# shicaiwei123/ICCV2025-GDL

Measured on AMD Instinct MI355X. Metric: audio-visual samples/sec, CREMA-D DGL train step (whole job), higher is better.
Workload: dtype bf16; 1 GPU; CREMA-D DGL (main_dgl.py, ConcatFusion_DGL) ResNet18 a+v, spec 1x257x188 + frames 3x3x224x224, alpha=4, SGD lr 2e-3 mom .9 wd 1e-4, clip 40; per_gpu_batch=64, global_batch=64, parallelism=dp1, buckets=none

## Files before the change

iccv2025-gdl_amd/csrc/api.cpp:

```cpp
#include "ops.h"

using namespace gdl;

#ifdef GDL_TIMING
namespace gdl { extern unsigned long long* g_timing_buf; }
#endif
extern "C" {
GDL_API int gdl_debug_timing_buffer(void* buf) {
#ifdef GDL_TIMING
    gdl::g_timing_buf = (unsigned long long*)buf;
    return GDL_OK;
#else
    (void)buf;
    return GDL_ERR_ARG;
#endif
}


const char* gdl_last_error(void) { return last_error(); }
int gdl_version(void) { return 100; }

int gdl_device_info(int* cu_count, char* name, int name_len) {
    int dev = 0;
    hipError_t e = hipGetDevice(&dev);
// ... 14 lines not shown
    return conv_tiles_m(dtype, N, H, W, C, K, R, S, stride, pad);
}

size_t gdl_conv_table_bytes(int mode, int N, int H, int W, int R, int S, int stride, int pad) {
    return gather_table_bytes(mode, N, H, W, R, S, stride, pad);
}
int gdl_conv_build_table(int mode, int dtype, int N, int H, int W, int C, int K, int R, int S, int stride, int pad,
                         void* table, void* stream) {
    GDL_REQUIRE(dt_ok(dtype) && table && (mode == GATHER_FWD || mode == GATHER_DGRAD), "conv_build_table: bad arguments");
    return build_gather_table(mode, dtype, N, H, W, C, K, R, S, stride, pad, (GatherEntry*)table, (hipStream_t)stream);
}
int gdl_conv_fwd(int dtype, const void* x, const void* w_krsc, void* y, float* bn_partial, const void* table, int N, int H,
                 int W, int C, int K, int R, int S, int stride, int pad, void* stream) {
    GDL_REQUIRE(x && w_krsc && y, "conv_fwd: null pointer");
    return conv_fwd(dtype, x, w_krsc, y, bn_partial, table, N, H, W, C, K, R, S, stride, pad, (hipStream_t)stream);
}
int gdl_bn_act_bits(int dtype, const void* y, const float* scale, const float* shift, const void* res, const float* res_scale,
                    const float* res_shift, void* out, uint8_t* relu_bits, size_t M, int C, void* stream) {
    GDL_REQUIRE(dt_ok(dtype) && y && scale && shift && out && relu_bits, "bn_act_bits: bad arguments");
    return bn_act(dtype, y, scale, shift, res, res_scale, res_shift, 1, out, M, C, (hipStream_t)stream, relu_bits);
}
int gdl_conv_dgrad_relu(int dtype, const void* dy, const void* w_crsk, void* dx, const void* addend, const uint8_t* relu_bits,
                        const void* table, int N, int H, int W, int C, int K, int R, int S, int stride, int pad, void* stream) {
    GDL_REQUIRE(dy && w_crsk && dx && relu_bits, "conv_dgrad_relu: null pointer");
    return conv_dgrad(dtype, dy, w_crsk, dx, addend, table, N, H, W, C, K, R, S, stride, pad, (hipStream_t)stream, relu_bits);
}
int gdl_conv_fwd_bias(int dtype, const void* x, const void* w_krsc, void* y, const float* bias, const void* addend, void* gelu_out,
                      const void* table, int N, int H, int W, int C, int K, int R, int S, int stride, int pad, void* stream) {
    GDL_REQUIRE(x && w_krsc && y, "conv_fwd_bias: null pointer");
    return conv_fwd_bias(dtype, x, w_krsc, y, bias, addend, gelu_out, table, N, H, W, C, K, R, S, stride, pad, (hipStream_t)stream);
// ... 628 lines not shown
```

iccv2025-gdl_amd/csrc/conv_igemm.hip:

```cpp
#include <stdlib.h>

#include <type_traits>

#include "bnacc.h"
#include "common.h"
#include "gather.h"
#include "ops.h"
#include "prof.h"

#include <hip/hip_ext.h>

namespace gdl {

struct ConvArgs {
    const void* in;
    const void* wt;
    void* out;
    const void* addend;
    const float* bias;
    void* gelu_out;
    const void* gelu_u;
    const uint8_t* relu_bits;
    float* stats;
    BnAcc sacc;
// ... 1048 lines not shown
        d[0] = acc_wait;
        d[1] = acc_issue;
        d[2] = acc_rd;
        d[3] = acc_m0;
        d[4] = acc_m1;
        d[5] = (unsigned long long)kpt * a.ntaps;
    }
#endif
}

#include "conv_pslab.h"

constexpr int C64_BM = 128;
constexpr int C64_GRID = 512;
constexpr int C64_F32_TILE = 35 * 1024;
template <int MODE, bool BW = false, bool ADD = false>
__global__ __launch_bounds__(256, 2) void conv3x3_c64_kernel(ConvArgs a) {
    static_assert(!BW || MODE == MODE_DGRAD, "BW: data gradient only");
    static_assert(!ADD || MODE == MODE_DGRAD, "ADD: data gradient only");
    constexpr bool STATS = MODE == MODE_FWD;
    extern __shared__ __attribute__((aligned(16))) unsigned char smem[];
    constexpr int BM = C64_BM, PITCH = 64 * 2 + 16;
    const int tid = threadIdx.x, lane = tid & 63, wave = __builtin_amdgcn_readfirstlane(tid >> 6);
    const int wm = wave & 1, wn = wave >> 1;
    const int frow = lane & 15, fg = lane >> 4;
    GDL_STAMP(0);
    const int xcd = blockIdx.x & 7, bj = blockIdx.x >> 3, bpx = gridDim.x >> 3;
    const int mt_per_xcd = (a.mtiles + 7) >> 3;
    const int t_end = min(a.mtiles, (xcd + 1) * mt_per_xcd);
    int tile = xcd * mt_per_xcd + bj;
    const int nins = (a.slab_rows + 7) >> 3;
    const int slab_bytes = BW ? max(nins * 1024, C64_F32_TILE) : nins * 1024;
    const unsigned smem_base = lds_addr(smem);
    const int nbuf = a.single_slab ? 1 : 2;
    const unsigned zrow = smem_base + nbuf * slab_bytes;
    const __amdgpu_buffer_rsrc_t rin = __builtin_amdgcn_make_buffer_rsrc((void*)a.in, 0, a.in_bytes, 0x00020000);

    typedef unsigned u32x4_t __attribute__((ext_vector_type(4)));
    u32x4_t wreg[9][2][2];
    {
        const __amdgpu_buffer_rsrc_t rwt = __builtin_amdgcn_make_buffer_rsrc((void*)a.wt, 0, a.wt_bytes, 0x00020000);
        for (int p = wave; p < 72; p += 4) {
            const int row = p * 8 + (lane >> 3);
            dma16(rwt, smem + p * 1024, row * 128 + (((lane & 7) ^ swz128(row)) << 4));
        }
        asm volatile("s_waitcnt vmcnt(0)" ::: "memory");
        __builtin_amdgcn_s_barrier();
        asm volatile("" ::: "memory");
#pragma unroll
        for (int tap = 0; tap < 9; ++tap)
#pragma unroll
            for (int h = 0; h < 2; ++h)
#pragma unroll
                for (int n = 0; n < 2; ++n) {
                    const int row = (wn * 32 + n * 16 + frow) * 9 + tap;
                    const unsigned ad = smem_base + row * 128 + (((h * 4 + fg) ^ swz128(row)) << 4);
                    asm volatile("ds_read_b128 %0, %1" : "=v"(wreg[tap][h][n]) : "v"(ad));
                }
        asm volatile("s_waitcnt lgkmcnt(0)" ::: "memory");
        __builtin_amdgcn_s_barrier();
        asm volatile("" ::: "memory");
    }
    if constexpr (BW) {
        if (tid < 128) ((float*)(smem + nbuf * slab_bytes + 1024))[tid] = tid < 64 ? a.bw_mean[tid] : a.bw_rstd[tid - 64];
        ((float*)(smem + nbuf * slab_bytes + 1536))[tid] = 0.f;
        ((float*)(smem + nbuf * slab_bytes + 1536))[tid + 256] = 0.f;
    }
    if (wave == 0) dma16(rin, smem + nbuf * slab_bytes, (int)0x80000000);
    auto load_slab = [&](int sbuf, int m0) {
        unsigned char* dst = smem + sbuf * slab_bytes;
        int ln = lane;
        asm volatile("" : "+v"(ln));
        for (int jj = wave; jj < nins; jj += 4) {
            const int sr = jj * 8 + (ln >> 3);
            const int pix = m0 - (a.W + 1) + sr;
            const bool ok = sr < a.slab_rows && (unsigned)pix < (unsigned)a.in_pixels;
            const int v = ok ? pix * 128 + (((ln & 7) ^ swz128(sr)) << 4) : (int)0x80000000;
            dma16(rin, dst + jj * 1024, v);
        }
    };
    auto load_masks = [&](int m0, unsigned (&fm)[4]) {
#pragma unroll
        for (int m = 0; m < 4; ++m) {
            const int mm = m0 + wm * 64 + m * 16 + frow;
            fm[m] = mm < a.M ? a.table[mm].mask : 0u;
        }
    };
    const int prow0 = wm * 64 + frow + (a.W + 1);
    unsigned zb[4];
#pragma unroll
    for (int m = 0; m < 4; ++m) zb[m] = zrow - 2048u * m;
    const int ec = tid & 7, er0 = tid >> 3;
    float tsum[8], tsq[8];
#pragma unroll
    for (int e = 0; e < 8; ++e) tsum[e] = tsq[e] = 0.f;
    bf16* __restrict__ gout = (bf16*)a.out;
    const bf16* __restrict__ gadd = ADD ? (const bf16*)a.addend : nullptr;
    const uint8_t* __restrict__ rbits = MODE == MODE_DGRAD ? a.relu_bits : nullptr;

    unsigned fmask[4] = {0u, 0u, 0u, 0u};
// ... 21 lines not shown
    GDL_STAMP(1);
#else
#define C64_SEG(i)
#endif
    for (int it = 0; tile < t_end; ++it, tile += bpx) {
#ifdef GDL_TIMING
        tq_a = __builtin_amdgcn_s_memtime();
        ++tq_n;
#endif
        const int m0 = tile * BM;
        const bool more = tile + bpx < t_end;
        const int sb = nbuf == 2 ? (it & 1) : 0;
        if (more && nbuf == 2) {
            load_slab(sb ^ 1, (tile + bpx) * BM);
        }
        C64_SEG(0)
        const unsigned slab = smem_base + sb * slab_bytes;
        f32x4_t acc[2][4];
#pragma unroll
        for (int n = 0; n < 2; ++n)
#pragma unroll
            for (int m = 0; m < 4; ++m) acc[n][m] = f32x4_t{0.f, 0.f, 0.f, 0.f};
        constexpr int NPX = STATS ? 1 : 2;
        uint4 px[NPX][4];
        unsigned pb[4];
        auto tap_addr = [&](int tap) __attribute__((always_inline)) {
            const int sr0 = prow0 + a.pshift[tap];
            const unsigned ad0 = slab + sr0 * 128 + ((fg ^ swz128(sr0)) << 4);
#pragma unroll
            for (int m = 0; m < 4; ++m) pb[m] = ((fmask[m] >> tap) & 1u) ? ad0 : zb[m];
// ... 261 lines not shown
                red[(wave * 64 + lane * 8 + e) * 2 + 1] = ssq[e];
            }
        }
        __syncthreads();
        if (tid < 128) {
            const int c = tid >> 1, w = tid & 1;
            const float s2 = ((red[(0 * 64 + c) * 2 + w] + red[(1 * 64 + c) * 2 + w]) + red[(2 * 64 + c) * 2 + w]) +
                             red[(3 * 64 + c) * 2 + w];
            if (a.sacc.acc)
                bn_acc_add(a.sacc, c, w, s2);
            else
                st_agent(sdst + ((size_t)blockIdx.x * 64 + c) * 2 + w, s2);
        }
    }
    GDL_STAMP(3);
}

static size_t slab_lds_bytes(int BM, int BN, int W, int IC, int dtype, bool single = false) {
    const int bke = dtype == GDL_BF16 ? 64 : 32, esz = dtype == GDL_BF16 ? 2 : 4;
    const int rows = BM + 2 * W + 2;
    const size_t slab = (size_t)((rows + 7) / 8) * 1024;
    const size_t main = 2 * (size_t)BN * 128 + ((IC / bke > 1 && !single) ? 2 : 1) * slab + ((rows & 7) ? 0 : 1024);
    const size_t epi = (size_t)BM * (BN * esz + 16) + 8 * (size_t)BN * 2 * 4;
    return main > epi ? main : epi;
}

struct TileCfg {
    int bm, bn;
};

// ... 21 lines not shown
    int split;
    int rows;
};
struct ConvOpts {
    const void* addend = nullptr;
    float* stats = nullptr;
    const uint8_t* relu_bits = nullptr;
    const void* dy_ds = nullptr;
    const void* w_ds = nullptr;
    const float* bias = nullptr;
    void* gelu_out = nullptr;
    const void* gelu_u = nullptr;
    const BwdStats* bw = nullptr;
    const BnAcc* sacc = nullptr;
    const SplitWs* split = nullptr;
};

static size_t c64_lds_bytes(int W, bool single = false) {
    const size_t b = (single ? 1 : 2) * (size_t)((C64_BM + 2 * W + 2 + 7) / 8) * 1024 + 1024 + 512 + 2048;
    return b > (size_t)72 * 1024 ? b : (size_t)72 * 1024;
}
static constexpr long slab_big_min() { return 128; }
static constexpr long slab_bn128_min() { return 384; }
constexpr int SPLITK_BLOCKS = 200;
static_assert(SPLITK_BLOCKS <= PS_GRID, "split-K blocks");
static int pslab_mode() {
    static int v = -1;
    if (v < 0) {
        const char* e = tune_env("GDL_PSLAB");
        v = e ? atoi(e) : 2;
// ... 164 lines not shown
        if (need > lds) lds = need;
        GDL_REQUIRE(lds <= (size_t)80 * 1024, "conv: LDS of the 64-channel data gradient with BatchNorm sums");
    }
    auto kfn = conv3x3_c64_kernel<MODE, BW, ADD>;
    static DevOnce attr_set;
    if (!attr_set) {
        hipError_t e = hipFuncSetAttribute((const void*)kfn, hipFuncAttributeMaxDynamicSharedMemorySize, 80 * 1024);
        if (e != hipSuccess) return check_hip(e, "hipFuncSetAttribute(conv3x3_c64)");
        attr_set = true;
    }
    static char pname[64] = "";
    if (!pname[0]) snprintf(pname, sizeof(pname), BW ? "gdl::conv3x3_c64_kernel<%d, true>" : "gdl::conv3x3_c64_kernel<%d>", MODE);
    ProfScope prof(pname, PROF_MFMA, st, a.flops, true, a.hbm_bytes);
    hipExtLaunchKernelGGL(kfn, dim3(C64_GRID), dim3(256), lds, st, prof.e0(), prof.e1(), 0, a);
    GDL_CHECK_LAUNCH("conv3x3_c64_kernel");
    return GDL_OK;
}

template <typename T, int MODE>
static int launch_mode(ConvArgs& a, const ConvPlan& pl, hipStream_t st) {
    constexpr bool BF = std::is_same<T, bf16>::value;
    switch (pl.kind) {
        case ConvKind::C64:
            if constexpr (BF) return launch_c64<MODE>(a, pl.lds, st);
            break;
        case ConvKind::PSLAB:
            if constexpr (BF) {
                if (pl.nslab == 1) return pl.bm == 192 ? launch_pslab<3, MODE, false>(a, pl, st) : launch_pslab<2, MODE, false>(a, pl, st);
                return pl.bm == 192 ? launch_pslab<3, MODE, true>(a, pl, st) : launch_pslab<2, MODE, true>(a, pl, st);
            }
// ... 210 lines not shown
    } else {
        a.IC = K;
        a.OC = C;
        a.in_bytes = (unsigned)((size_t)N * P * Q * K * esz);
    }
    a.wt_bytes = (unsigned)((size_t)K * C * R * S * esz);
    GDL_REQUIRE(a.IC % bke == 0, "conv: gather channels %d not a multiple of %d", a.IC, bke);
    GDL_REQUIRE(a.OC % 64 == 0, "conv: output channels %d not a multiple of 64", a.OC);
    GDL_REQUIRE(a.M < (1 << 24), "conv: M = %d exceeds 2^24", a.M);
    if (a.plain && !o.stats && !sacc && !o.relu_bits && !bw && !o.gelu_u && !o.dy_ds &&
        linear_stream_ok(dtype, a.M, a.IC, a.OC, o.addend != nullptr))
        return linear_stream_fwd(in, wt, out, o.addend, o.bias, o.gelu_out, a.M, a.IC, a.OC, st);
    ConvPlan pl;
    rc = plan_conv(pl, mode, dtype, N, H, W, C, K, R, S, stride, pad, o);
    if (rc) return rc;
    a.flops = 2.0 * (double)N * P * Q * K * C * R * S;
    {
        const double esz = dtype == GDL_BF16 ? 2.0 : 4.0;
        a.hbm_bytes = esz * ((double)N * H * W * C + (double)N * P * Q * K + (double)K * C * R * S);
    }
    if (o.dy_ds) {
        GDL_REQUIRE(mode == GATHER_DGRAD && stride == 2 && R == 3 && S == 3 && pad == 1 && o.w_ds && pl.kind == ConvKind::FLAT,
                    "conv: the folded downsample branch needs the 3x3 stride-2 pad-1 data gradient");
        a.in2 = o.dy_ds;
        a.wt2 = o.w_ds;
        a.in2_bytes = a.in_bytes;
        a.wt2_bytes = (unsigned)((size_t)K * C * esz);
        a.flops += 2.0 * (double)N * P * Q * K * C;
    }
    if (mode == GATHER_DGRAD && stride == 2) {
// ... 29 lines not shown
        f.bw_y = a.bw_y, f.bw_mean = a.bw_mean, f.bw_rstd = a.bw_rstd, f.bw_partial = a.bw_partial;
        f.bw_y2 = a.bw_y2, f.bw_mean2 = a.bw_mean2, f.bw_rstd2 = a.bw_rstd2, f.bw_partial2 = a.bw_partial2;
        ProfScope prof("gdl::splitk_finish_kernel", PROF_HBM, st, (double)a.M * a.OC * (4.0 * ks + 2.0 * (1 + (a.addend ? 1 : 0) + (a.bw_y ? 1 : 0) + (a.bw_y2 ? 1 : 0))));
        hipLaunchKernelGGL(splitk_finish_kernel<bf16>, dim3(mt, a.OC / 64), dim3(256), 0, st, f);
        GDL_CHECK_LAUNCH("splitk_finish_kernel");
        if (pl.rows > mt) {
            const size_t off = (size_t)mt * a.OC * 2, n = (size_t)(pl.rows - mt) * a.OC * 2 * sizeof(float);
            for (float* p : {a.stats, a.bw_partial, a.bw_y2 ? a.bw_partial2 : (float*)nullptr})
                if (p) {
                    hipError_t e = hipMemsetAsync(p + off, 0, n, st);
                    if (e != hipSuccess) return check_hip(e, "hipMemsetAsync(split-K partial rows)");
                }
        }
        return GDL_OK;
    }
    if (dtype == GDL_BF16)
        return mode == GATHER_FWD ? launch_mode<bf16, MODE_FWD>(a, pl, st) : launch_mode<bf16, MODE_DGRAD>(a, pl, st);
    return mode == GATHER_FWD ? launch_mode<float, MODE_FWD>(a, pl, st) : launch_mode<float, MODE_DGRAD>(a, pl, st);
}

int conv_fwd(int dtype, const void* x, const void* w, void* y, float* bn_partial, const void* table, int N, int H, int W,
             int C, int K, int R, int S, int stride, int pad, hipStream_t st, const BnAcc* sacc, const SplitWs* split) {
    ConvOpts o;
    o.stats = bn_partial, o.sacc = sacc, o.split = split;
    return run_conv(GATHER_FWD, dtype, x, w, y, table, N, H, W, C, K, R, S, stride, pad, st, o);
}

int stem_taps(int dtype);
int stem_ic(int dtype);
static bool stem_rows(int dtype, int W) {
    static int v = -1;
    if (v < 0) {
        const char* e = tune_env("GDL_STEM_ROWS_FWD");
        v = e ? atoi(e) : 1;
    }
    return v != 0 && dtype == GDL_BF16 && (W - 1) / 2 + 1 >= 64;
}
static bool stem_pers() {
    static int v = -1;
    if (v < 0) {
// ... 124 lines not shown
```

iccv2025-gdl_amd/csrc/encoder.cpp:

```cpp
#include <map>
#include <tuple>
#include <vector>

#include "ops.h"

using namespace gdl;

namespace {

struct Conv {
    int cin, cout, r, s, stride, pad;
    int h, w, p, q;
    int pidx;
    void* w_krsc = nullptr;
    void* w_crsk = nullptr;
    void* tab_fwd = nullptr;
    void* tab_dgrad = nullptr;
};
struct BN {
    int c;
    int pidx;
    int bidx;
    float *scale = nullptr, *shift = nullptr, *mean = nullptr, *rstd = nullptr, *coef = nullptr;
    long long* acc = nullptr;
// ... 415 lines not shown
    if (he == hipSuccess) he = hipStreamSynchronize((hipStream_t)stream);
    if (he != hipSuccess) return -check_hip(he, "encoder_bn_overflow: read-back");
    int n = 0;
    auto flagged = [&](const BN& b) {
        if (b.acc && host[(size_t)(b.acc - e->acc_arena) + 2 * (size_t)b.c] != 0) ++n;
    };
    flagged(e->bn0);
    for (const Block& k : e->blocks) {
        flagged(k.b1);
        flagged(k.b2);
        if (k.has_ds) flagged(k.bd);
    }
    return n;
}

#define RC(x)                 \
    do {                      \
        int rc__ = (x);       \
        if (rc__) return rc__; \
    } while (0)

#ifdef GDL_EXPERIMENT
static unsigned skip_mask() {
    static long v = -1;
    if (v < 0) {
        const char* env = getenv("GDL_SKIP");
        v = env ? atol(env) : 0;
    }
    return (unsigned)v;
}
// ... 40 lines not shown
}

static bool separate_stats() {
    static int sep = -1;
    if (sep < 0) {
        const char* env = tune_env("GDL_SEPARATE_STATS");
        sep = env ? atoi(env) : 0;
    }
    return sep != 0;
}

static bool bn_acc_on() {
    static int v = -1;
    if (v < 0) {
        const char* env = tune_env("GDL_BN_ACC");
        v = env ? atoi(env) : 1;
    }
    return v != 0;
}
static BnAcc acc_producer(const BN& n, size_t rows) {
    BnAcc a{n.acc, 0.0, 0.0, n.acc ? n.acc + 2 * (size_t)n.c : nullptr};
    bn_acc_scales(rows, &a.s1, &a.s2);
    return a;
}
static BnAccFin acc_consumer(gdl_encoder* e, BN& n, size_t rows) {
    double s1, s2;
    bn_acc_scales(rows, &s1, &s2);
    return BnAccFin{n.acc, 1.0 / s1, 1.0 / s2, (double)rows, e->params[n.pidx], e->params[n.pidx + 1], e->rmean[n.bidx],
                    e->rvar[n.bidx], e->nbt[n.bidx], n.mean, n.rstd, n.scale, n.shift, 1e-5f, 0.1f,
                    n.acc ? n.acc + 2 * (size_t)n.c : nullptr};
// ... 92 lines not shown
                               e->h0, e->w0, 64, st, &f0));
    }
    for (Block& k : e->blocks) {
        const size_t Mo = (size_t)k.n * k.p * k.q;
        if (acc) {
            auto conv = [&](const Conv& c, const BN& n, const void* x, void* y) {
                if (c.stride == 1 && c.r == 3 && (GDL_SKIPPED(65536) || (GDL_SKIPPED(2048) && c.cout == 512))) return (int)GDL_OK;
                if ((c.stride == 2 || c.r == 1) && GDL_SKIPPED(32768)) return (int)GDL_OK;
                if (c.r == 1 && GDL_SKIPPED(2097152)) return (int)GDL_OK;
                const BnAcc pa = acc_producer(n, Mo);
                return conv_fwd(dt, x, c.w_krsc, y, nullptr, c.tab_fwd, k.n, c.h, c.w, c.cin, c.cout, c.r, c.s, c.stride, c.pad, st,
                                &pa, &e->sk);
            };
            RC(conv(k.c1, k.b1, k.xin, k.y1));
            const BnAccFin f1 = acc_consumer(e, k.b1, Mo), f2 = acc_consumer(e, k.b2, Mo);
            RC(bn_act(dt, k.y1, k.b1.scale, k.b1.shift, nullptr, nullptr, nullptr, 1, k.a1, Mo, k.cout, st,
                      bw_fuse_on() ? k.abits : nullptr, &f1));
            RC(conv(k.c2, k.b2, k.a1, k.y2));
            if (k.has_ds) {
                RC(conv(k.cd, k.bd, k.xin, k.yd));
                const BnAccFin fd = acc_consumer(e, k.bd, Mo);
                RC(bn_act(dt, k.y2, k.b2.scale, k.b2.shift, k.yd, k.bd.scale, k.bd.shift, 1, k.z, Mo, k.cout, st, k.zbits, &f2, &fd));
            } else {
                RC(bn_act(dt, k.y2, k.b2.scale, k.b2.shift, k.xin, nullptr, nullptr, 1, k.z, Mo, k.cout, st, k.zbits, &f2));
            }
            continue;
        }
        RC(conv_bn(e, k.c1, k.b1, k.xin, k.y1, k.n, training, st));
        if (!(GDL_SKIPPED(1) || (GDL_SKIPPED(2) && k.cout == 64)))
            RC(bn_act(dt, k.y1, k.b1.scale, k.b1.shift, nullptr, nullptr, nullptr, 1, k.a1, Mo, k.cout, st,
                      (training && bw_fuse_on()) ? k.abits : nullptr));
        if (k.has_ds && training && !separate_stats()) {
            auto fin = [&](const Conv& c, BN& n, const float* partial) {
// ... 278 lines not shown
```

iccv2025-gdl_amd/csrc/ops.h:

```cpp
#pragma once
#include "bnacc.h"
#include "common.h"
#include "gather.h"

namespace gdl {

const char* last_error();

struct BnFinTrain {
    const float* partial;
    int tiles, C;
    double count;
    const float *gamma, *beta;
    float *running_mean, *running_var;
    int64_t* nbt;
    float *save_mean, *save_rstd, *scale, *shift;
};
struct BnFinBwd {
    const float* partial;
    int blocks, C;
    double count;
    float *dgamma, *dbeta, *coef;
};

// ... 6 lines not shown
    float* partial2;
};
struct SplitWs {
    void* ptr;
    size_t bytes;
};
size_t conv_split_ws_bytes(int dtype, int N, int H, int W, int C, int K, int R, int S, int stride, int pad, int dgrad);
bool linear_stream_ok(int dtype, int M, int K, int N, bool has_addend);
int linear_stream_fwd(const void* A, const void* W, void* out, const void* addend, const float* bias, void* gelu_out, int M, int K,
                      int N, hipStream_t st);
int conv_dgrad_tiles_m(int dtype, int N, int H, int W, int C, int K, int R, int S, int stride, int pad);
int conv_tiles_m(int dtype, int N, int H, int W, int C, int K, int R, int S, int stride, int pad);
int conv_fwd(int dtype, const void* x, const void* w_krsc, void* y, float* bn_partial, const void* table, int N, int H,
             int W, int C, int K, int R, int S, int stride, int pad, hipStream_t st, const BnAcc* sacc = nullptr,
             const SplitWs* split = nullptr);
int conv_fwd_bias(int dtype, const void* x, const void* w_krsc, void* y, const float* bias, const void* addend, void* gelu_out,
                  const void* table, int N, int H, int W, int C, int K, int R, int S, int stride, int pad, hipStream_t st);
int conv_dgrad(int dtype, const void* dy, const void* w_crsk, void* dx, const void* addend, const void* table, int N, int H,
               int W, int C, int K, int R, int S, int stride, int pad, hipStream_t st, const uint8_t* relu_bits = nullptr,
               const BwdStats* bw = nullptr, const SplitWs* split = nullptr);
int conv_dgrad_gelu(int dtype, const void* dy, const void* w_crsk, void* dx, const void* u, const BnAcc* acc, const void* table,
                    int N, int H, int W, int C, int K, int R, int S, int stride, int pad, hipStream_t st);
int acc_to_float(const long long* acc, int n, double inv_scale, float* out, hipStream_t st);
int conv_dgrad_ds(int dtype, const void* dy, const void* w_crsk, const void* dy_ds, const void* w_ds_ck, void* dx,
                  const void* table, int N, int H, int W, int C, int K, hipStream_t st, const uint8_t* relu_bits = nullptr,
                  const BwdStats* bw = nullptr);
size_t stem_pad_bytes(int dtype, int n_img, int H, int W);
int stem_taps(int dtype);
int stem_ic(int dtype);
int stem_pad(int dtype, const float* x, void* xp, int B, int Cin, int T, int H, int W, hipStream_t st, void* zero = nullptr,
// ... 192 lines not shown
```

iccv2025-gdl_amd/gdl/_lib.py:

```python
import ctypes
import os

_HERE = os.path.dirname(os.path.abspath(__file__))
SO_PATH = os.environ.get("GDL_LIB") or os.path.join(os.path.dirname(_HERE), "csrc", "build", "libgdl_hip.so")

GDL_F32, GDL_BF16 = 0, 1
GDL_AUDIO, GDL_VISUAL = 0, 1
GATHER_FWD, GATHER_DGRAD = 0, 1
GDL_LAYOUT_NHWC, GDL_LAYOUT_NCHW = 0, 1
ENC_NPARAMS, ENC_NBN = 60, 20
GDL_JOURNAL_COLS = 16

_C = {"i": ctypes.c_int, "p": ctypes.c_void_p, "z": ctypes.c_size_t, "f": ctypes.c_float, "d": ctypes.c_double,
      "l": ctypes.c_int64, "s": ctypes.c_char_p}

SIGNATURES = {
    "gdl_last_error": ("s", ""),
    "gdl_version": ("i", ""),
    "gdl_device_info": ("i", "ppi"),
    "gdl_conv_bn_tiles": ("i", "iiiiiiiiii"),
    "gdl_conv_table_bytes": ("z", "iiiiiiii"),
    "gdl_conv_build_table": ("i", "ii" + "iiiiiiiii" + "pp"),
    "gdl_conv_fwd": ("i", "ippppp" + "iiiiiiiii" + "p"),
    "gdl_conv_dgrad": ("i", "ippppp" + "iiiiiiiii" + "p"),
    "gdl_bn_act_bits": ("i", "ippp" + "ppp" + "pp" + "zi" + "p"),
    "gdl_conv_dgrad_relu": ("i", "ipppppp" + "iiiiiiiii" + "p"),
    "gdl_conv_fwd_bias": ("i", "ippppppp" + "iiiiiiiii" + "p"),
    "gdl_conv_dgrad_ds": ("i", "ippppppp" + "iiiii" + "p"),
    "gdl_conv_dgrad_bn_tiles": ("i", "iiiiiiiiii"),
    "gdl_conv_dgrad_bn": ("i", "ipppppp" + "iiiiiiiii" + "pppppppp" + "p"),
    "gdl_conv_split_workspace_bytes": ("z", "iiiiiiiiiii"),
    "gdl_conv_fwd_split": ("i", "ippppp" + "iiiiiiiii" + "pz" + "p"),
    "gdl_conv_dgrad_bn_split": ("i", "ipppppp" + "iiiiiiiii" + "pppppppp" + "pz" + "p"),
    "gdl_conv_dgrad_gelu": ("i", "ippppp" + "d" + "p" + "iiiiiiiii" + "p"),
    "gdl_acc_to_float": ("i", "pidpp"),
    "gdl_comm_unique_id": ("i", "p"),
    "gdl_comm_init": ("i", "piip"),
    "gdl_comm_world": ("i", "p"),
    "gdl_comm_allreduce_bucket": ("i", "ppz" + "p"),
# ... 123 lines not shown
    "gdl_dul_eval": ("i", "pppppp" + "ii" + "p"),
    "gdl_encoder_create": ("i", "piiiiii"),
    "gdl_encoder_destroy": (None, "p"),
    "gdl_encoder_side_stream": ("i", "pi"),
    "gdl_encoder_borrow_side_stream": ("i", "pp"),
    "gdl_encoder_backward_phase": ("i", "pippp" + "p"),
    "gdl_encoder_workspace_bytes": ("z", "p"),
    "gdl_encoder_param_numel": ("i", "pp"),
    "gdl_encoder_out_shape": ("i", "pppp"),
    "gdl_encoder_bind": ("i", "ppz"),
    "gdl_encoder_set_params": ("i", "ppppp"),
    "gdl_encoder_forward": ("i", "ppippp"),
    "gdl_encoder_backward": ("i", "ppppp"),
    "gdl_encoder_forward_serial": ("l", "p"),
    "gdl_encoder_bn_overflow": ("i", "pp"),
    "gdl_prof_enable": ("i", "i"),
    "gdl_prof_enabled": ("i", ""),
    "gdl_prof_set_filter": ("i", "s"),
    "gdl_debug_timing_buffer": ("i", "p"),
    "gdl_prof_nslots": ("i", ""),
    "gdl_prof_slot_name": ("s", "i"),
    "gdl_prof_slot_bound": ("i", "i"),
    "gdl_prof_collect": ("i", "ppp"),
    "gdl_prof_set_peaks": ("i", "dd"),
    "gdl_prof_collect_floor": ("i", "pp"),
    "gdl_prof_timeline": ("i", "ipppppp"),
    "gdl_stem_bwd_fused_ok": ("i", "ii"),
    "gdl_stem_bwd_fused": ("i", "ipppppppppp" + "p" + "iiii" + "pz" + "p"),
}

# ... 66 lines not shown
```

include/gdl_hip.h:

```cpp
#ifndef GDL_HIP_H
#define GDL_HIP_H
#include <stddef.h>
#include <stdint.h>

#ifdef __cplusplus
extern "C" {
#endif

#define GDL_API __attribute__((visibility("default")))

enum { GDL_OK = 0, GDL_ERR_ARG = 1, GDL_ERR_HIP = 2, GDL_ERR_STATE = 3, GDL_ERR_WORKSPACE = 4 };
enum { GDL_F32 = 0, GDL_BF16 = 1 };
enum { GDL_AUDIO = 0, GDL_VISUAL = 1 };

GDL_API const char* gdl_last_error(void);
GDL_API int gdl_version(void);
GDL_API int gdl_device_info(int* cu_count, char* name, int name_len);

enum { GDL_GATHER_FWD = 0, GDL_GATHER_DGRAD = 1 };
GDL_API size_t gdl_conv_table_bytes(int mode, int N, int H, int W, int R, int S, int stride, int pad);
GDL_API int gdl_conv_build_table(int mode, int dtype, int N, int H, int W, int C, int K, int R, int S, int stride,
                                 int pad, void* table, void* stream);
GDL_API int gdl_conv_bn_tiles(int dtype, int N, int H, int W, int C, int K, int R, int S, int stride, int pad);
GDL_API int gdl_conv_fwd(int dtype, const void* x, const void* w_krsc, void* y, float* bn_partial, const void* table,
                         int N, int H, int W, int C, int K, int R, int S, int stride, int pad, void* stream);
GDL_API int gdl_conv_dgrad(int dtype, const void* dy, const void* w_crsk, void* dx, const void* addend,
                           const void* table, int N, int H, int W, int C, int K, int R, int S, int stride, int pad,
                           void* stream);
GDL_API int gdl_bn_act_bits(int dtype, const void* y, const float* scale, const float* shift, const void* res,
                            const float* res_scale, const float* res_shift, void* out, uint8_t* relu_bits, size_t M, int C,
                            void* stream);
GDL_API int gdl_conv_dgrad_relu(int dtype, const void* dy, const void* w_crsk, void* dx, const void* addend,
                                const uint8_t* relu_bits, const void* table, int N, int H, int W, int C, int K, int R, int S,
                                int stride, int pad, void* stream);
GDL_API int gdl_conv_fwd_bias(int dtype, const void* x, const void* w_krsc, void* y, const float* bias, const void* addend,
                              void* gelu_out, const void* table, int N, int H, int W, int C, int K, int R, int S, int stride,
                              int pad, void* stream);
GDL_API int gdl_conv_dgrad_ds(int dtype, const void* dy, const void* w_crsk, const void* dy_ds, const void* w_ds_ck, void* dx,
                              const uint8_t* relu_bits, const void* table, int N, int H, int W, int C, int K, void* stream);
GDL_API int gdl_conv_dgrad_bn_tiles(int dtype, int N, int H, int W, int C, int K, int R, int S, int stride, int pad);
GDL_API int gdl_conv_dgrad_bn(int dtype, const void* dy, const void* w_crsk, void* dx, const void* addend,
                              const uint8_t* relu_bits, const void* table, int N, int H, int W, int C, int K, int R, int S,
                              int stride, int pad, const void* y, const float* mean, const float* rstd, float* partial,
// ... 205 lines not shown
GDL_API int gdl_encoder_borrow_side_stream(gdl_encoder_t* e, void* stream);
GDL_API size_t gdl_encoder_workspace_bytes(const gdl_encoder_t* e);
GDL_API int gdl_encoder_param_numel(const gdl_encoder_t* e, int64_t* numel );
GDL_API int gdl_encoder_out_shape(const gdl_encoder_t* e, int* n_img, int* h, int* w);
GDL_API int gdl_encoder_bind(gdl_encoder_t* e, void* workspace, size_t bytes);
GDL_API int gdl_encoder_set_params(gdl_encoder_t* e, const float* const* params, float* const* running_mean,
                                   float* const* running_var, int64_t* const* num_batches_tracked);
GDL_API int gdl_encoder_forward(gdl_encoder_t* e, const float* x, int training, float* feat_out, float* fmap_nchw,
                                void* stream);
GDL_API int gdl_encoder_backward(gdl_encoder_t* e, const float* dfeat, const float* dfmap_nchw, float* const* grads,
                                 void* stream);
GDL_API int gdl_encoder_backward_phase(gdl_encoder_t* e, int phase, const float* dfeat, const float* dfmap_nchw,
                                       float* const* grads, void* stream);
GDL_API int64_t gdl_encoder_forward_serial(const gdl_encoder_t* e);
GDL_API int gdl_encoder_bn_overflow(gdl_encoder_t* e, void* stream);

#define GDL_LAYOUT_NHWC 0
#define GDL_LAYOUT_NCHW 1
GDL_API size_t gdl_feature_diversity_workspace_bytes(int n_img);
GDL_API int gdl_feature_diversity(const void* map, int dtype, int layout, int n_img, int P, int C, float* per_image,
                                  float* mean_out, float* accum, void* ws, size_t ws_bytes, void* stream);
GDL_API int gdl_encoder_feature_diversity(gdl_encoder_t* e, float* per_image, float* mean_out, float* accum, void* ws,
                                          size_t ws_bytes, void* stream);

#define GDL_JOURNAL_COLS 16
GDL_API size_t gdl_journal_bytes(int64_t capacity);
GDL_API int gdl_journal_append(void* journal, int64_t capacity, const float* losses, int n_losses, const float* stats,
                               const float* out_a, const float* out_v, int64_t n_logits, const float* div_a, const float* div_v,
                               const float* ogm, void* stream);

// ... 87 lines not shown
```

Before: 13180 samples/s.

## Fuse BatchNorm+ReLU of first conv into 64-channel 3x3 conv input slab

Adds a variant of the 64-channel 3x3 conv kernel that applies the preceding BatchNorm scale/shift and ReLU to the input slab in LDS. It also writes out the activated tensor and ReLU bitmask from inside the kernel. In the basic-block forward pass this replaces the separate bn_act launch and its full read of y1 before conv2, when the shape is eligible (enabled by default via GDL_C64_XBN). Halo rows are transformed redundantly across tiles, and per-tile work adds LDS read/write passes that may lengthen the conv's critical path.

```diff
diff --git a/iccv2025-gdl_amd/csrc/api.cpp b/iccv2025-gdl_amd/csrc/api.cpp
--- a/iccv2025-gdl_amd/csrc/api.cpp
+++ b/iccv2025-gdl_amd/csrc/api.cpp
@@ -52,6 +52,14 @@
                  int W, int C, int K, int R, int S, int stride, int pad, void* stream) {
     GDL_REQUIRE(x && w_krsc && y, "conv_fwd: null pointer");
     return conv_fwd(dtype, x, w_krsc, y, bn_partial, table, N, H, W, C, K, R, S, stride, pad, (hipStream_t)stream);
+}
+int gdl_conv_fwd_bnin_tiles(void) { return conv_fwd_xbn_rows(); }
+int gdl_conv_fwd_bnin(int dtype, const void* x, const float* scale, const float* shift, const void* w_krsc, void* y, void* a_out,
+                      uint8_t* relu_bits_out, float* bn_partial, const void* table, int N, int H, int W, int C, int K,
+                      void* stream) {
+    GDL_REQUIRE(dt_ok(dtype) && x && scale && shift && w_krsc && y && a_out && table, "conv_fwd_bnin: null pointer");
+    return conv_fwd_xbn(dtype, x, scale, shift, nullptr, w_krsc, y, a_out, relu_bits_out, bn_partial, table, N, H, W, C, K,
+                        (hipStream_t)stream);
 }
 int gdl_bn_act_bits(int dtype, const void* y, const float* scale, const float* shift, const void* res, const float* res_scale,
                     const float* res_shift, void* out, uint8_t* relu_bits, size_t M, int C, void* stream) {
diff --git a/iccv2025-gdl_amd/csrc/conv_igemm.hip b/iccv2025-gdl_amd/csrc/conv_igemm.hip
--- a/iccv2025-gdl_amd/csrc/conv_igemm.hip
+++ b/iccv2025-gdl_amd/csrc/conv_igemm.hip
@@ -1086,10 +1086,17 @@
 constexpr int C64_BM = 128;
 constexpr int C64_GRID = 512;
 constexpr int C64_F32_TILE = 35 * 1024;
-template <int MODE, bool BW = false, bool ADD = false>
-__global__ __launch_bounds__(256, 2) void conv3x3_c64_kernel(ConvArgs a) {
+struct XbnArgs {
+    const float *scale, *shift;
+    BnAccFin fin;
+    void* a_out;
+    uint8_t* bits;
+};
+template <int MODE, bool BW, bool ADD, bool XBN>
+__device__ __forceinline__ void conv3x3_c64_body(const ConvArgs& a, const XbnArgs& xb) {
     static_assert(!BW || MODE == MODE_DGRAD, "BW: data gradient only");
     static_assert(!ADD || MODE == MODE_DGRAD, "ADD: data gradient only");
+    static_assert(!XBN || MODE == MODE_FWD, "XBN: forward only");
     constexpr bool STATS = MODE == MODE_FWD;
     extern __shared__ __attribute__((aligned(16))) unsigned char smem[];
     constexpr int BM = C64_BM, PITCH = 64 * 2 + 16;
@@ -1110,12 +1117,21 @@
 
     typedef unsigned u32x4_t __attribute__((ext_vector_type(4)));
     u32x4_t wreg[9][2][2];
+    float xsc = 0.f, xsf = 0.f;
     {
         const __amdgpu_buffer_rsrc_t rwt = __builtin_amdgcn_make_buffer_rsrc((void*)a.wt, 0, a.wt_bytes, 0x00020000);
         for (int p = wave; p < 72; p += 4) {
             const int row = p * 8 + (lane >> 3);
             dma16(rwt, smem + p * 1024, row * 128 + (((lane & 7) ^ swz128(row)) << 4));
         }
+        if constexpr (XBN) {
+            if (tid < 64) {
+                if (xb.fin.acc)
+                    bn_acc_channel(xb.fin, tid, blockIdx.x == 0, xsc, xsf);
+                else
+                    xsc = xb.scale[tid], xsf = xb.shift[tid];
+            }
+        }
         asm volatile("s_waitcnt vmcnt(0)" ::: "memory");
         __builtin_amdgcn_s_barrier();
         asm volatile("" ::: "memory");
@@ -1137,6 +1153,12 @@
         if (tid < 128) ((float*)(smem + nbuf * slab_bytes + 1024))[tid] = tid < 64 ? a.bw_mean[tid] : a.bw_rstd[tid - 64];
         ((float*)(smem + nbuf * slab_bytes + 1536))[tid] = 0.f;
         ((float*)(smem + nbuf * slab_bytes + 1536))[tid + 256] = 0.f;
+    }
+    if constexpr (XBN) {
+        if (tid < 64) {
+            ((float*)(smem + nbuf * slab_bytes + 1024))[tid] = xsc;
+            ((float*)(smem + nbuf * slab_bytes + 1024))[64 + tid] = xsf;
+        }
     }
     if (wave == 0) dma16(rin, smem + nbuf * slab_bytes, (int)0x80000000);
     auto load_slab = [&](int sbuf, int m0) {
@@ -1156,6 +1178,67 @@
         for (int m = 0; m < 4; ++m) {
             const int mm = m0 + wm * 64 + m * 16 + frow;
             fm[m] = mm < a.M ? a.table[mm].mask : 0u;
+        }
+    };
+    auto xbn_apply = [&](int sbuf, int m0) __attribute__((always_inline)) {
+        if constexpr (XBN) {
+            int t = tid;
+            asm volatile("" : "+v"(t));
+            const int r0 = t >> 3, lc = (t & 7) ^ swz128(r0);
+            const unsigned cad = smem_base + nbuf * slab_bytes + 1024 + lc * 32;
+            u32x4_t c0, c1, c2, c3;
+            asm volatile("ds_read_b128 %0, %1" : "=v"(c0) : "v"(cad));
+            asm volatile("ds_read_b128 %0, %1 offset:16" : "=v"(c1) : "v"(cad));
+            asm volatile("ds_read_b128 %0, %1 offset:256" : "=v"(c2) : "v"(cad));
+            asm volatile("ds_read_b128 %0, %1 offset:272" : "=v"(c3) : "v"(cad));
+            asm volatile("s_waitcnt lgkmcnt(0)" ::: "memory");
+            asm volatile("" : "+v"(c0), "+v"(c1), "+v"(c2), "+v"(c3));
+            const float sc[8] = {__uint_as_float(c0.x), __uint_as_float(c0.y), __uint_as_float(c0.z), __uint_as_float(c0.w),
+                                 __uint_as_float(c1.x), __uint_as_float(c1.y), __uint_as_float(c1.z), __uint_as_float(c1.w)};
+            const float sf[8] = {__uint_as_float(c2.x), __uint_as_float(c2.y), __uint_as_float(c2.z), __uint_as_float(c2.w),
+                                 __uint_as_float(c3.x), __uint_as_float(c3.y), __uint_as_float(c3.z), __uint_as_float(c3.w)};
+            bf16* __restrict__ ga = (bf16*)xb.a_out;
+            uint8_t* __restrict__ gb = xb.bits;
+            unsigned ad = smem_base + sbuf * slab_bytes + r0 * 128 + ((t & 7) << 4);
+            for (int r = r0; r < a.slab_rows; r += 128, ad += 4 * 4096) {
+                u32x4_t v[4];
+                const unsigned ad1 = r + 32 < a.slab_rows ? ad + 4096u : ad, ad2 = r + 64 < a.slab_rows ? ad + 8192u : ad,
+                               ad3 = r + 96 < a.slab_rows ? ad + 12288u : ad;
+                asm volatile("ds_read_b128 %0, %1" : "=v"(v[0]) : "v"(ad));
+                asm volatile("ds_read_b128 %0, %1" : "=v"(v[1]) : "v"(ad1));
+                asm volatile("ds_read_b128 %0, %1" : "=v"(v[2]) : "v"(ad2));
+                asm volatile("ds_read_b128 %0, %1" : "=v"(v[3]) : "v"(ad3));
+                asm volatile("s_waitcnt lgkmcnt(0)" ::: "memory");
+                asm volatile("" : "+v"(v[0]), "+v"(v[1]), "+v"(v[2]), "+v"(v[3]));
+#pragma unroll
+                for (int j = 0; j < 4; ++j) {
+                    float f[8];
+                    unpack16<bf16>(make_uint4(v[j].x, v[j].y, v[j].z, v[j].w), f);
+                    unsigned mk = 0u;
+#pragma unroll
+                    for (int e = 0; e < 8; ++e) {
+                        float x = f[e] * sc[e] + sf[e];
+                        x = x > 0.f ? x : 0.f;
+                        f[e] = x;
+                        mk |= (x > 0.f ? 1u : 0u) << e;
+                    }
+                    const uint4 o = pack16<bf16>(f);
+                    v[j] = u32x4_t{o.x, o.y, o.z, o.w};
+                    const int q = r + 32 * j - (a.W + 1);
+                    if ((unsigned)q < (unsigned)BM && m0 + q < a.M) {
+                        const size_t vec = (size_t)(m0 + q) * 8 + lc;
+                        *(uint4*)(ga + vec * 8) = o;
+                        if (gb) gb[vec] = (uint8_t)mk;
+                    }
+                }
+                asm volatile("ds_write_b128 %0, %1" ::"v"(ad), "v"(v[0]) : "memory");
+                if (r + 32 < a.slab_rows) asm volatile("ds_write_b128 %0, %1 offset:4096" ::"v"(ad), "v"(v[1]) : "memory");
+                if (r + 64 < a.slab_rows) asm volatile("ds_write_b128 %0, %1 offset:8192" ::"v"(ad), "v"(v[2]) : "memory");
+                if (r + 96 < a.slab_rows) asm volatile("ds_write_b128 %0, %1 offset:12288" ::"v"(ad), "v"(v[3]) : "memory");
+            }
+            asm volatile("s_waitcnt lgkmcnt(0)" ::: "memory");
+            __builtin_amdgcn_s_barrier();
+            asm volatile("" ::: "memory");
         }
     };
     const int prow0 = wm * 64 + frow + (a.W + 1);
@@ -1207,6 +1290,7 @@
         if (more && nbuf == 2) {
             load_slab(sb ^ 1, (tile + bpx) * BM);
         }
+        xbn_apply(sb, m0);
         C64_SEG(0)
         const unsigned slab = smem_base + sb * slab_bytes;
         f32x4_t acc[2][4];
@@ -1498,6 +1582,13 @@
         }
     }
     GDL_STAMP(3);
+}
+template <int MODE, bool BW = false, bool ADD = false>
+__global__ __launch_bounds__(256, 2) void conv3x3_c64_kernel(ConvArgs a) {
+    conv3x3_c64_body<MODE, BW, ADD, false>(a, XbnArgs{});
+}
+__global__ __launch_bounds__(256, 2) void conv3x3_c64_xbn_kernel(ConvArgs a, XbnArgs xb) {
+    conv3x3_c64_body<MODE_FWD, false, false, true>(a, xb);
 }
 
 static size_t slab_lds_bytes(int BM, int BN, int W, int IC, int dtype, bool single = false) {
@@ -1549,6 +1640,7 @@
     const BwdStats* bw = nullptr;
     const BnAcc* sacc = nullptr;
     const SplitWs* split = nullptr;
+    const XbnArgs* xbn = nullptr;
 };
 
 static size_t c64_lds_bytes(int W, bool single = false) {
@@ -1743,6 +1835,24 @@
     ProfScope prof(pname, PROF_MFMA, st, a.flops, true, a.hbm_bytes);
     hipExtLaunchKernelGGL(kfn, dim3(C64_GRID), dim3(256), lds, st, prof.e0(), prof.e1(), 0, a);
     GDL_CHECK_LAUNCH("conv3x3_c64_kernel");
+    return GDL_OK;
+}
+
+static int launch_c64_xbn(ConvArgs& a, const XbnArgs& xb, size_t lds, hipStream_t st) {
+    a.mtiles = ceil_div(a.M, C64_BM);
+    GDL_REQUIRE(!a.bias && !a.gelu_out && !a.orow && !a.addend && !a.relu_bits && a.ksplit <= 1,
+                "conv: unsupported option for the 64-channel kernel with BatchNorm on its input");
+    GDL_REQUIRE(lds <= (size_t)80 * 1024, "conv: LDS of the 64-channel kernel with BatchNorm on its input");
+    auto kfn = conv3x3_c64_xbn_kernel;
+    static DevOnce attr_set;
+    if (!attr_set) {
+        hipError_t e = hipFuncSetAttribute((const void*)kfn, hipFuncAttributeMaxDynamicSharedMemorySize, 80 * 1024);
+        if (e != hipSuccess) return check_hip(e, "hipFuncSetAttribute(conv3x3_c64_xbn)");
+        attr_set = true;
+    }
+    ProfScope prof("gdl::conv3x3_c64_xbn_kernel", PROF_MFMA, st, a.flops, true, a.hbm_bytes + 2.0 * (double)a.M * 64);
+    hipExtLaunchKernelGGL(kfn, dim3(C64_GRID), dim3(256), lds, st, prof.e0(), prof.e1(), 0, a, xb);
+    GDL_CHECK_LAUNCH("conv3x3_c64_xbn_kernel");
     return GDL_OK;
 }
 
@@ -1983,6 +2093,10 @@
     ConvPlan pl;
     rc = plan_conv(pl, mode, dtype, N, H, W, C, K, R, S, stride, pad, o);
     if (rc) return rc;
+    if (o.xbn) {
+        const int nslab = c64_lds_bytes(W) > (size_t)80 * 1024 ? 1 : 2;
+        pl = ConvPlan{ConvKind::C64, C64_BM, 64, nslab, c64_lds_bytes(W, nslab == 1), C64_GRID, 1, C64_GRID};
+    }
     a.flops = 2.0 * (double)N * P * Q * K * C * R * S;
     {
         const double esz = dtype == GDL_BF16 ? 2.0 : 4.0;
@@ -2042,6 +2156,7 @@
         }
         return GDL_OK;
     }
+    if (o.xbn) return launch_c64_xbn(a, *o.xbn, pl.lds, st);
     if (dtype == GDL_BF16)
         return mode == GATHER_FWD ? launch_mode<bf16, MODE_FWD>(a, pl, st) : launch_mode<bf16, MODE_DGRAD>(a, pl, st);
     return mode == GATHER_FWD ? launch_mode<float, MODE_FWD>(a, pl, st) : launch_mode<float, MODE_DGRAD>(a, pl, st);
@@ -2052,6 +2167,30 @@
     ConvOpts o;
     o.stats = bn_partial, o.sacc = sacc, o.split = split;
     return run_conv(GATHER_FWD, dtype, x, w, y, table, N, H, W, C, K, R, S, stride, pad, st, o);
+}
+
+int conv_fwd_xbn_rows() { return C64_GRID; }
+static bool c64_serves(int W) {
+    return c64_lds_bytes(W, true) <= (size_t)80 * 1024 && (size_t)((C64_BM + 2 * W + 2 + 7) / 8) * 1024 >= (size_t)C64_BM * 144;
+}
+bool conv_fwd_xbn_planned(int dtype, int N, int H, int W, int C, int K) {
+    return C == 64 && K == 64 && geometry_plan(GATHER_FWD, dtype, N, H, W, C, K, 3, 3, 1, 1).kind == ConvKind::C64;
+}
+int conv_fwd_xbn(int dtype, const void* x, const float* scale, const float* shift, const BnAccFin* fin, const void* w, void* y,
+                 void* a_out, uint8_t* relu_bits_out, float* bn_partial, const void* table, int N, int H, int W, int C, int K,
+                 hipStream_t st, const BnAcc* sacc) {
+    GDL_REQUIRE(x && w && y && a_out, "conv_fwd_xbn: null pointer");
+    GDL_REQUIRE(dtype == GDL_BF16, "conv_fwd_xbn: bf16 only");
+    GDL_REQUIRE(C == 64 && K == 64, "conv_fwd_xbn: %d -> %d channels, the fused kernel serves 64 -> 64", C, K);
+    GDL_REQUIRE(N > 0 && H > 0 && W > 0 && c64_serves(W), "conv_fwd_xbn: image width %d outside the fused kernel's range", W);
+    const bool acc = fin && fin->acc;
+    GDL_REQUIRE(acc || (scale && shift), "conv_fwd_xbn: neither scale / shift arrays nor accumulators");
+    XbnArgs xb{};
+    xb.scale = scale, xb.shift = shift, xb.a_out = a_out, xb.bits = relu_bits_out;
+    if (acc) xb.fin = *fin;
+    ConvOpts o;
+    o.stats = bn_partial, o.sacc = sacc, o.xbn = &xb;
+    return run_conv(GATHER_FWD, dtype, x, w, y, table, N, H, W, C, K, 3, 3, 1, 1, st, o);
 }
 
 int stem_taps(int dtype);
diff --git a/iccv2025-gdl_amd/csrc/encoder.cpp b/iccv2025-gdl_amd/csrc/encoder.cpp
--- a/iccv2025-gdl_amd/csrc/encoder.cpp
+++ b/iccv2025-gdl_amd/csrc/encoder.cpp
@@ -453,6 +453,25 @@
     return n;
 }
 
+int gdl_encoder_bn_saved(gdl_encoder_t* e, int index, float* mean, float* rstd, float* scale, float* shift, void* stream) {
+    if (!e || !e->ws || !mean || !rstd || !scale || !shift || index < 0) return -GDL_ERR_ARG;
+    std::vector<const BN*> all{&e->bn0};
+    for (const Block& k : e->blocks) {
+        all.push_back(&k.b1);
+        all.push_back(&k.b2);
+        if (k.has_ds) all.push_back(&k.bd);
+    }
+    if ((size_t)index >= all.size()) return -GDL_ERR_ARG;
+    const BN& b = *all[index];
+    const size_t n = sizeof(float) * b.c;
+    const std::pair<float*, const float*> cp[4] = {{mean, b.mean}, {rstd, b.rstd}, {scale, b.scale}, {shift, b.shift}};
+    for (const auto& p : cp) {
+        hipError_t he = hipMemcpyAsync(p.first, p.second, n, hipMemcpyDeviceToDevice, (hipStream_t)stream);
+        if (he != hipSuccess) return -check_hip(he, "encoder_bn_saved: copy");
+    }
+    return b.c;
+}
+
 #define RC(x)                 \
     do {                      \
         int rc__ = (x);       \
@@ -523,6 +542,14 @@
     static int v = -1;
     if (v < 0) {
         const char* env = tune_env("GDL_BN_ACC");
+        v = env ? atoi(env) : 1;
+    }
+    return v != 0;
+}
+static bool c64_xbn_on() {
+    static int v = -1;
+    if (v < 0) {
+        const char* env = tune_env("GDL_C64_XBN");
         v = env ? atoi(env) : 1;
     }
     return v != 0;
@@ -645,9 +672,18 @@
             };
             RC(conv(k.c1, k.b1, k.xin, k.y1));
             const BnAccFin f1 = acc_consumer(e, k.b1, Mo), f2 = acc_consumer(e, k.b2, Mo);
-            RC(bn_act(dt, k.y1, k.b1.scale, k.b1.shift, nullptr, nullptr, nullptr, 1, k.a1, Mo, k.cout, st,
-                      bw_fuse_on() ? k.abits : nullptr, &f1));
-            RC(conv(k.c2, k.b2, k.a1, k.y2));
+            const Conv& c2 = k.c2;
+            if (dt == GDL_BF16 && c64_xbn_on() && c2.stride == 1 && c2.r == 3 && !GDL_SKIPPED(65536) &&
+                conv_fwd_xbn_planned(dt, k.n, c2.h, c2.w, c2.cin, c2.cout)) {
+                const BnAcc pa = acc_producer(k.b2, Mo);
+                RC(conv_fwd_xbn(dt, k.y1, nullptr, nullptr, &f1, c2.w_krsc, k.y2, k.a1, bw_fuse_on() ? k.abits : nullptr, nullptr,
+                                c2.tab_fwd, k.n, c2.h, c2.w, c2.cin, c2.cout, st, &pa));
+            } else {
+                if (!(GDL_SKIPPED(1) || (GDL_SKIPPED(2) && k.cout == 64)))
+                    RC(bn_act(dt, k.y1, k.b1.scale, k.b1.shift, nullptr, nullptr, nullptr, 1, k.a1, Mo, k.cout, st,
+                              bw_fuse_on() ? k.abits : nullptr, &f1));
+                RC(conv(k.c2, k.b2, k.a1, k.y2));
+            }
             if (k.has_ds) {
                 RC(conv(k.cd, k.bd, k.xin, k.yd));
                 const BnAccFin fd = acc_consumer(e, k.bd, Mo);
diff --git a/iccv2025-gdl_amd/csrc/ops.h b/iccv2025-gdl_amd/csrc/ops.h
--- a/iccv2025-gdl_amd/csrc/ops.h
+++ b/iccv2025-gdl_amd/csrc/ops.h
@@ -44,6 +44,11 @@
 int conv_fwd(int dtype, const void* x, const void* w_krsc, void* y, float* bn_partial, const void* table, int N, int H,
              int W, int C, int K, int R, int S, int stride, int pad, hipStream_t st, const BnAcc* sacc = nullptr,
              const SplitWs* split = nullptr);
+int conv_fwd_xbn(int dtype, const void* x, const float* scale, const float* shift, const BnAccFin* fin, const void* w_krsc,
+                 void* y, void* a_out, uint8_t* relu_bits_out, float* bn_partial, const void* table, int N, int H, int W, int C,
+                 int K, hipStream_t st, const BnAcc* sacc = nullptr);
+int conv_fwd_xbn_rows();
+bool conv_fwd_xbn_planned(int dtype, int N, int H, int W, int C, int K);
 int conv_fwd_bias(int dtype, const void* x, const void* w_krsc, void* y, const float* bias, const void* addend, void* gelu_out,
                   const void* table, int N, int H, int W, int C, int K, int R, int S, int stride, int pad, hipStream_t st);
 int conv_dgrad(int dtype, const void* dy, const void* w_crsk, void* dx, const void* addend, const void* table, int N, int H,
diff --git a/iccv2025-gdl_amd/gdl/_lib.py b/iccv2025-gdl_amd/gdl/_lib.py
--- a/iccv2025-gdl_amd/gdl/_lib.py
+++ b/iccv2025-gdl_amd/gdl/_lib.py
@@ -23,6 +23,8 @@
     "gdl_conv_build_table": ("i", "ii" + "iiiiiiiii" + "pp"),
     "gdl_conv_fwd": ("i", "ippppp" + "iiiiiiiii" + "p"),
     "gdl_conv_dgrad": ("i", "ippppp" + "iiiiiiiii" + "p"),
+    "gdl_conv_fwd_bnin_tiles": ("i", ""),
+    "gdl_conv_fwd_bnin": ("i", "ipppp" + "pppp" + "p" + "iiiii" + "p"),
     "gdl_bn_act_bits": ("i", "ippp" + "ppp" + "pp" + "zi" + "p"),
     "gdl_conv_dgrad_relu": ("i", "ipppppp" + "iiiiiiiii" + "p"),
     "gdl_conv_fwd_bias": ("i", "ippppppp" + "iiiiiiiii" + "p"),
@@ -176,6 +178,7 @@
     "gdl_encoder_backward": ("i", "ppppp"),
     "gdl_encoder_forward_serial": ("l", "p"),
     "gdl_encoder_bn_overflow": ("i", "pp"),
+    "gdl_encoder_bn_saved": ("i", "pi" + "pppp" + "p"),
     "gdl_prof_enable": ("i", "i"),
     "gdl_prof_enabled": ("i", ""),
     "gdl_prof_set_filter": ("i", "s"),
diff --git a/include/gdl_hip.h b/include/gdl_hip.h
--- a/include/gdl_hip.h
+++ b/include/gdl_hip.h
@@ -27,6 +27,10 @@
 GDL_API int gdl_conv_dgrad(int dtype, const void* dy, const void* w_crsk, void* dx, const void* addend,
                            const void* table, int N, int H, int W, int C, int K, int R, int S, int stride, int pad,
                            void* stream);
+GDL_API int gdl_conv_fwd_bnin_tiles(void);
+GDL_API int gdl_conv_fwd_bnin(int dtype, const void* x, const float* scale, const float* shift, const void* w_krsc, void* y,
+                              void* a_out, uint8_t* relu_bits_out, float* bn_partial, const void* table, int N, int H, int W,
+                              int C, int K, void* stream);
 GDL_API int gdl_bn_act_bits(int dtype, const void* y, const float* scale, const float* shift, const void* res,
                             const float* res_scale, const float* res_shift, void* out, uint8_t* relu_bits, size_t M, int C,
                             void* stream);
@@ -262,6 +266,8 @@
                                        float* const* grads, void* stream);
 GDL_API int64_t gdl_encoder_forward_serial(const gdl_encoder_t* e);
 GDL_API int gdl_encoder_bn_overflow(gdl_encoder_t* e, void* stream);
+GDL_API int gdl_encoder_bn_saved(gdl_encoder_t* e, int index, float* mean, float* rstd, float* scale, float* shift,
+                                 void* stream);
 
 #define GDL_LAYOUT_NHWC 0
 #define GDL_LAYOUT_NCHW 1
```

Result: faster. 13320 samples/s (median of 6 runs) (+1.1%).
